# rmcolq/charon

Measured on AMD Instinct MI355X. Metric: classified reads/sec + achieved HBM GB/s vs roofline, 5 kb reads, 39 GB index, higher is better.
Workload: dtype u64

## Files before the change

charon_amd/api.py:

```python
import ctypes as C
import os

import numpy as np

HERE = os.path.dirname(os.path.abspath(__file__))
LIB_PATH = os.environ.get("CHARON_HIP_LIB") or os.path.join(HERE, "libcharon_hip.so")
if not os.path.exists(LIB_PATH):
    raise ImportError("charon_amd: %s not built -- run `python -c 'import __graft_entry__ as g; g.build()'`" % LIB_PATH)
_L = C.CDLL(LIB_PATH)

MINIMISER_SEED = 0x8F3F73B5CF1C9ADE
STREAM_PROFILE = 1
STREAM_TINY_LOG = 2
GZIP_TALLIES, GZIP_SIZES, GZIP_BOTH = 0, 1, 2
GZIP_SIZES_ALL = 3
GZIP_ANY_LEN = 0xFFFFFFFF


class IndexDesc(C.Structure):
    _fields_ = [("struct_size", C.c_uint32), ("device", C.c_int32), ("kmer_size", C.c_uint8), ("window_size", C.c_uint8),
                ("hash_funs", C.c_uint8), ("num_categories", C.c_uint8), ("host_index", C.c_uint8), ("reserved0", C.c_uint8 * 3),
                ("minimiser_seed", C.c_uint64), ("bins", C.c_uint64), ("technical_bins", C.c_uint64), ("bin_size", C.c_uint64),
                ("hash_shift", C.c_uint64), ("bin_words", C.c_uint64), ("bin_to_category", C.c_uint8 * 256),
                ("row_begin", C.c_uint64), ("row_end", C.c_uint64)]


class Model(C.Structure):
    _fields_ = [("struct_size", C.c_uint32), ("num_categories", C.c_uint32), ("pos_data", C.POINTER(C.POINTER(C.c_float))),
                ("pos_n", C.POINTER(C.c_uint32)), ("neg_data", C.POINTER(C.POINTER(C.c_float))), ("neg_n", C.POINTER(C.c_uint32)),
                ("h_pos", C.c_float), ("h_neg", C.c_float), ("err_rate", C.c_float), ("min_quality", C.c_float),
                ("min_length", C.c_uint32), ("min_compression", C.c_float), ("confidence_threshold", C.c_int8),
                ("min_hits", C.c_uint8), ("paired", C.c_uint8), ("host_index", C.c_uint8),
                ("confidence_probability_threshold", C.c_float), ("host_unique_prop_lo_threshold", C.c_float),
                ("min_proportion_difference", C.c_float), ("min_prob_difference", C.c_float),
                ("dist", C.c_uint32), ("pos_params", C.POINTER(C.c_float)), ("neg_params", C.POINTER(C.c_float))]


class StreamCfg(C.Structure):
    _fields_ = [("struct_size", C.c_uint32), ("flags", C.c_uint32), ("max_reads", C.c_uint64), ("max_bases", C.c_uint64)]


class Batch(C.Structure):
    _fields_ = [("struct_size", C.c_uint32), ("on_device", C.c_uint32), ("n_reads", C.c_uint64), ("n_bases", C.c_uint64),
                ("bases2", C.c_void_p), ("nmask", C.c_void_p), ("seg1_offset", C.c_void_p), ("seg1_length", C.c_void_p),
                ("seg2_offset", C.c_void_p), ("seg2_length", C.c_void_p), ("mean_quality", C.c_void_p),
                ("compression", C.c_void_p), ("gzip_tallies", C.c_uint32), ("gzip_output", C.c_uint32)]
# ... 288 lines not shown

    def synth_fill(self, seed, density):
        _chk(_L.chn_synth_fill_index(self.h, seed, density))

    def synth_plant(self, dev_genomes, n_genomes, genome_len, genome_bin):
        _chk(_L.chn_synth_plant(self.h, dev_genomes, n_genomes, genome_len, bytes(bytearray(int(b) for b in genome_bin))))

    def destroy(self):
        if self.h:
            _L.chn_index_destroy(self.h)
            self.h = None


DIST = {"kde": 0, "gamma": 1, "beta": 2}
DIST_DEFAULTS = {"gamma": ((25.0, 0.0, 0.02), (10.0, 0.0, 0.005)), "beta": ((6.0, 4.0, 0.0), (6.0, 40.0, 0.0))}


def default_model(num_categories, host_index, paired=False, dist="kde", pos_params=None, neg_params=None, **overrides):
    m = Model()
    _chk(_L.chn_model_default(C.byref(m), num_categories, host_index, 1 if paired else 0))
    if dist != "kde":
        pp = np.ascontiguousarray(pos_params if pos_params is not None else [DIST_DEFAULTS[dist][0]] * num_categories, np.float32)
        nn = np.ascontiguousarray(neg_params if neg_params is not None else [DIST_DEFAULTS[dist][1]] * num_categories, np.float32)
        m._keep = (pp, nn)
        m.dist = DIST[dist]
        m.pos_params = pp.ctypes.data_as(C.POINTER(C.c_float))
        m.neg_params = nn.ctypes.data_as(C.POINTER(C.c_float))
    for k, v in overrides.items():
        setattr(m, k, v)
    return m


class Stream:
    def __init__(self, index, max_reads, max_bases, profile=False, tiny_log=False, split_bucket=0):
        self.index = index
        cfg = StreamCfg(C.sizeof(StreamCfg), (STREAM_PROFILE if profile else 0) | (STREAM_TINY_LOG if tiny_log else 0) | ((split_bucket & 0xff) << 8),
                        max_reads, max_bases)
        self.h = C.c_void_p()
        _chk(_L.chn_stream_create(index.h, C.byref(cfg), C.byref(self.h)))
        self.C = index.desc.num_categories
        self._fifo = []

    def set_model(self, model):
        _chk(_L.chn_model_set(self.h, C.byref(model)))

    def submit_host(self, packed, mean_quality=None, compression=None, gzip_tallies=0, gzip_output=0):
        b, keep, n = self._host_batch(packed, mean_quality, compression)
        b.gzip_tallies, b.gzip_output = gzip_tallies, gzip_output
        _chk(_L.chn_batch_submit(self.h, C.byref(b)))
        self._fifo.append((n, keep, gzip_tallies, gzip_output))

    def _host_batch(self, packed, mean_quality, compression):
        n = len(packed["seg1_length"])
        b = Batch()
        b.struct_size, b.on_device, b.n_reads, b.n_bases = C.sizeof(Batch), 0, n, packed["n_bases"]
        keep = []

        def ptr(a, dt):
            if a is None:
                return None
            a = np.ascontiguousarray(a, dtype=dt)
            keep.append(a)
            return a.ctypes.data

        b.bases2 = ptr(packed["bases2"], np.uint32)
        b.nmask = ptr(packed.get("nmask"), np.uint32)
        b.seg1_offset = ptr(packed["seg1_offset"], np.uint64)
        b.seg1_length = ptr(packed["seg1_length"], np.uint32)
        b.seg2_offset = ptr(packed.get("seg2_offset"), np.uint64)
# ... 638 lines not shown
```

charon_amd/csrc/parts/abi_index_model.inc:

```

struct chn_index {
    chn_index_desc d;
    uint64_t *words = nullptr;
    uint64_t rows_local = 0;
    bool single_bin_categories = false;
    hipStream_t ef_stream = nullptr;
    hipEvent_t ef_copied = nullptr;
    void *ef_buf[2][4] = {{nullptr, nullptr, nullptr, nullptr}, {nullptr, nullptr, nullptr, nullptr}};
    size_t ef_cap[2][4] = {{0, 0, 0, 0}, {0, 0, 0, 0}};
    unsigned long long *ef_bad = nullptr;
    unsigned ef_turn = 0;
    void ef_release() {
        if (ef_stream) (void)hipStreamSynchronize(ef_stream);
        for (int k = 0; k < 2; ++k)
            for (int i = 0; i < 4; ++i) { if (ef_buf[k][i]) (void)hipFree(ef_buf[k][i]); ef_buf[k][i] = nullptr; ef_cap[k][i] = 0; }
        if (ef_bad) (void)hipFree(ef_bad);
        ef_bad = nullptr;
        if (ef_copied) (void)hipEventDestroy(ef_copied);
        ef_copied = nullptr;
        if (ef_stream) (void)hipStreamDestroy(ef_stream);
        ef_stream = nullptr;
    }
};

// ... 136 lines not shown
    chn_stream_cfg cfg;
    hipStream_t stream = nullptr;
    hipStream_t stream1 = nullptr;
    hipStream_t stream2 = nullptr;
    hipStream_t stream0 = nullptr;
    hipStream_t stream3 = nullptr;
    hipStream_t stream4 = nullptr;
    hipStream_t stream5 = nullptr;
    uint32_t long_bucket = 104;
    DevBuf d_hist, d_model;
    DevBuf d_memo;
    LogBuf big;
    DevBuf d_list, d_cbase;
    uint64_t shard_entries = 0;
    bool shard_open = false;
    LogBuf shx;
    DevBuf d_shx_cnt;
    ShxArgs shx_args;
    int shx_stage = 0;
    uint32_t cap_num = 65536, esc_shift = 0;
    uint64_t overflow_reruns = 0;
    bool gzt_big_lds = false;
    DevBuf d_gzscratch;
    DevBuf d_gzlscratch[2];
    bool gzl_big_lds = false;
    uint32_t n_cus = 256;
    static const int N_SLOTS = 3;
    Slot slot[N_SLOTS];
    PinBuf h_block;
    int head = 0;
    int inflight = 0;
    uint64_t batch_seq = 0;
    bool last_had_long = false;
    HostModel model;
    K3Args k3;
    struct CountsBufs { DevBuf num_hashes, counts, unique, len1, mq, comp, prob, call, conf, flags; } cc;
    double prof_ms[4] = {0, 0, 0, 0};
    uint64_t prof_n[4] = {0, 0, 0, 0};
    hipEvent_t prof_anchor[2] = {nullptr, nullptr};
    int prof_cur = 0;
    bool prof_anchor_pending = false, prof_have_end = false;
    double prof_prev_end = 0;
    std::chrono::steady_clock::time_point prof_anchor_at;
    uint64_t last_bytes = 0, last_min = 0, last_fetches = 0;
    double text_ms[2] = {0, 0};
    uint64_t text_n = 0;
    TextSplitScratch tsp;
    TextFetchScratch txg;
    TextPairScratch tpi;
};

static uint64_t pow5(unsigned e) { uint64_t p = 1; while (e--) p *= 5; return p; }

extern "C" int chn_index_create(const chn_index_desc *desc, chn_index **out) {
    if (!desc || !out || desc->struct_size != sizeof(chn_index_desc)) return fail(CHN_E_INVALID, "chn_index_create: bad descriptor");
    const chn_index_desc &d = *desc;
    if (d.kmer_size < 1 || d.kmer_size > 27) return fail(CHN_E_INVALID, "kmer_size must be in 1..27 (5^k has to fit 64 bits)");
    if (d.window_size < d.kmer_size) return fail(CHN_E_INVALID, "window_size must be >= kmer_size");
    if (d.hash_funs < 1 || d.hash_funs > 5) return fail(CHN_E_INVALID, "hash_funs must be in 1..5");
    if (d.bins < 1 || d.bins > 255 || d.technical_bins != ((d.bins + 63) / 64) * 64 || d.bin_words != d.technical_bins / 64)
        return fail(CHN_E_INVALID, "IBF header inconsistent: technical_bins must be 64*ceil(bins/64), bin_words = technical_bins/64");
    if (d.bin_size == 0 || d.hash_shift != (uint64_t)__builtin_clzll(d.bin_size)) return fail(CHN_E_INVALID, "hash_shift must be countl_zero(bin_size)");
    if (d.num_categories < 1) return fail(CHN_E_INVALID, "num_categories must be >= 1");
    for (uint64_t b = 0; b < d.bins; ++b)
        if (d.bin_to_category[b] >= d.num_categories) return fail(CHN_E_INVALID, "bin_to_category entry out of range");
    chn_index *idx = new (std::nothrow) chn_index();
// ... 283 lines not shown
```

charon_amd/csrc/parts/abi_shard_wait.inc:

```

static int ensure_shard_buffers(chn_stream *s) {
    const uint64_t nw = (s->cfg.max_reads + WAVE - 1) / WAVE;
    int rc;
    if ((rc = s->big.ensure(s->cfg.max_bases, nw, (uint32_t)s->idx->d.bin_words, 65536, 0))) return rc;
    if ((rc = s->d_list.ensure(s->big.log_cap * 8)) || (rc = s->d_cbase.ensure((nw + 1) * 8))) return rc;
    return CHN_OK;
}
static ShardArgs shard_args(chn_stream *s, const chn_index *shard, uint64_t *partial, const Slot &sl) {
    ShardArgs a;
    std::memset(&a, 0, sizeof a);
    const chn_index_desc &d = shard->d;
    a.list = s->d_list.as<uint64_t>(); a.wave_meta = s->big.meta.as<WaveMeta>(); a.cbase = s->d_cbase.as<uint64_t>();
    a.wave_count = s->big.wcount.as<uint32_t>(); a.words = shard->words; a.S = d.bin_size; a.row_begin = d.row_begin; a.row_end = d.row_end;
    a.shift = (uint32_t)d.hash_shift; a.h = d.hash_funs; a.W = (uint32_t)d.bin_words; a.partial = partial; a.rows = s->big.rows.as<uint64_t>();
    a.rowlog = s->big.log.as<uint32_t>(); a.B = (uint32_t)d.bins;
    a.n_waves = (uint32_t)((sl.n_reads + WAVE - 1) / WAVE); a.esc_capacity = s->big.esc_cap;
    a.status = reinterpret_cast<uint32_t *>(const_cast<Slot &>(sl).d_ctl.as<unsigned long long>() + CTL_STATUS);
    return a;
}

extern "C" int chn_shard_minimise(chn_stream *s, const chn_batch *b, uint64_t *n_entries) {
    if (!s || !b || !n_entries) return fail(CHN_E_INVALID, "chn_shard_minimise: null argument");
    if (s->shard_open) return fail(CHN_E_STATE, "chn_shard_minimise: previous sharded batch not finished");
    HIPCHK(hipSetDevice(s->idx->d.device));
// ... 103 lines not shown
    HIPCHK(hipStreamWaitEvent(s->stream2, sl.k1_done, 0));
    int rc = launch_tail(s, sl, s->big, s->stream2);
    if (rc) return rc;
    s->head = (s->head + 1) % chn_stream::N_SLOTS;
    s->inflight += 1;
    return CHN_OK;
}

extern "C" int chn_stream_sync(chn_stream *s) {
    if (!s) return fail(CHN_E_INVALID, "null stream");
    HIPCHK(hipSetDevice(s->idx->d.device));
    HIPCHK(hipStreamSynchronize(s->stream0));
    HIPCHK(hipStreamSynchronize(s->stream));
    HIPCHK(hipStreamSynchronize(s->stream1));
    HIPCHK(hipStreamSynchronize(s->stream4));
    HIPCHK(hipStreamSynchronize(s->stream2));
    return CHN_OK;
}

static int rerun_worst_case(chn_stream *s, Slot &sl) {
    const chn_index_desc &d = s->idx->d;
    unsigned long long *ctl = sl.d_ctl.as<unsigned long long>();
    const uint64_t n = sl.n_reads, nw = (n + WAVE - 1) / WAVE + sl.split_bound;
    HIPCHK(hipMemsetAsync(ctl, 0, CTL_NLONG * 8, s->stream));
    HIPCHK(hipMemsetAsync(ctl + CTL_FETCHES, 0, (CTL_WORDS - CTL_FETCHES) * 8, s->stream));
    hipLaunchKernelGGL(k_sum_len, dim3((uint32_t)std::min<uint64_t>(1024, (n + 255) / 256)), dim3(256), 0, s->stream, sl.len1, sl.len2, (uint32_t)n, ctl + CTL_WORDS - 1);
    HIPCHK(hipGetLastError());
    unsigned long long total = 0;
    HIPCHK(hipMemcpyAsync(&total, ctl + CTL_WORDS - 1, 8, hipMemcpyDeviceToHost, s->stream));
    HIPCHK(hipStreamSynchronize(s->stream));
    int rc = s->big.ensure(total, (n + WAVE - 1) / WAVE + std::min<uint64_t>(sl.split_bound, total / len_bucket_floor(std::min(s->long_bucket, 247u)) + 1), (uint32_t)d.bin_words, 65536, 0, nw);
    if (rc) return rc;
    K1Args a = sl.k1;
    fill_k1_log(a, sl, s->big, true);
    const size_t lds = k1_lds_bytes(a.wn, d.num_categories, MODE_ROWS, a.h, (uint32_t)d.bin_words, (uint32_t)d.bins);
    hipError_t e = launch_k1_mode(MODE_ROWS, (uint32_t)d.bin_words, a, lds, s->stream);
    if (e == hipSuccess && sl.split_bound) e = launch_k1_split_mode(MODE_ROWS, (uint32_t)d.bin_words, a, lds, s->stream, split_grid(sl.split_bound));
    if (e != hipSuccess) return fail(CHN_E_HIP, std::string("k_minimise_probe re-run: ") + hipGetErrorString(e));
    if ((rc = launch_tail(s, sl, s->big, s->stream))) return rc;
    HIPCHK(hipStreamSynchronize(s->stream));
    s->overflow_reruns += 1;
    return CHN_OK;
}

extern "C" int chn_batch_wait(chn_stream *s, chn_result *r) {
    if (!s || !r || r->struct_size != sizeof(chn_result)) return fail(CHN_E_INVALID, "chn_batch_wait: bad argument");
    if (s->inflight == 0) return fail(CHN_E_STATE, "no batch in flight");
    HIPCHK(hipSetDevice(s->idx->d.device));
    Slot &sl = s->slot[(s->head + chn_stream::N_SLOTS - s->inflight) % chn_stream::N_SLOTS];
    static const bool diag_wait = diag_env("CHN_DIAG_WAIT") != nullptr;
    auto dnow = []() { return std::chrono::duration<double>(std::chrono::steady_clock::now().time_since_epoch()).count(); };
    const double dw0 = diag_wait ? dnow() : 0;
    HIPCHK(hipEventSynchronize(sl.done));
    const double dw1 = diag_wait ? dnow() : 0;
    if (sl.want_gzt) HIPCHK(hipEventSynchronize(sl.gz_done));
    const double dw2 = diag_wait ? dnow() : 0;
    struct DiagPrint { bool on; double a, b, c; std::function<double()> now; ~DiagPrint() { if (on) std::fprintf(stderr, "chn_batch_wait: at %.4f  done-event %.2f ms  gz-event %.2f ms  rest %.2f ms\n", a, (b - a) * 1e3, (c - b) * 1e3, (now() - c) * 1e3); } } diag_print{diag_wait, dw0, dw1, dw2, dnow};
    s->inflight -= 1;
    static const int evpair[4][2] = {{0, 1}, {2, 3}, {4, 5}, {6, 7}};
    for (int i = 0; i < 4; ++i)
        if (sl.ev_used[i]) {
            float ms = 0;
            HIPCHK(hipEventElapsedTime(&ms, sl.ev[evpair[i][0]], sl.ev[evpair[i][1]]));
            if (i == 0) {
                float t0 = 0, t1 = 0;
                HIPCHK(hipEventElapsedTime(&t0, s->prof_anchor[s->prof_cur], sl.ev[0]));
// ... 111 lines not shown
    k3.mean_quality = mean_quality ? b.mq.as<float>() : nullptr; k3.compression = compression ? b.comp.as<float>() : nullptr;
    k3.prob = b.prob.as<double>(); k3.call = b.call.as<uint8_t>(); k3.conf = b.conf.as<uint8_t>(); k3.flags = b.flags.as<uint8_t>();
    k3.n_reads = (uint32_t)n;
    hipLaunchKernelGGL(k_model_call, dim3((uint32_t)((n + 255) / 256)), dim3(256), 0, s->stream, k3);
    HIPCHK(hipGetLastError());
    HIPCHK(hipStreamSynchronize(s->stream));
    HIPCHK(hipMemcpy(probabilities, b.prob.p, n * C * 8, hipMemcpyDeviceToHost));
    HIPCHK(hipMemcpy(call, b.call.p, n, hipMemcpyDeviceToHost));
    HIPCHK(hipMemcpy(confidence, b.conf.p, n, hipMemcpyDeviceToHost));
    HIPCHK(hipMemcpy(flags, b.flags.p, n, hipMemcpyDeviceToHost));
    return CHN_OK;
}

extern "C" int chn_classify_counts(chn_stream *s, uint64_t n, const uint32_t *num_hashes, const uint32_t *counts,
                                   const uint32_t *unique_counts, const uint32_t *lengths, const float *mean_quality,
                                   const float *compression, double *probabilities, uint8_t *call, uint8_t *confidence) {
    std::vector<uint8_t> flags(std::max<uint64_t>(n, 1));
    int rc = chn_classify_counts_raw(s, n, num_hashes, counts, unique_counts, lengths, mean_quality, compression, probabilities, call,
                                     confidence, flags.data());
    if (rc) return rc;
    const uint64_t C = s->idx->d.num_categories;
    std::vector<double> p(C);
    const bool all = s->model.dist != CHN_DIST_KDE;
    for (uint64_t i = 0; i < n; ++i)
        if (all || flags[i] || num_hashes[i] == 0) {
            host_model_call(s->model, num_hashes[i], counts + i * C, unique_counts + i * C, mean_quality ? mean_quality[i] : 0.0f,
                            compression ? compression[i] : 0.0f, lengths[i], p.data(), &call[i], &confidence[i]);
            for (uint64_t c = 0; c < C; ++c) probabilities[i * C + c] = p[c];
        }
    return CHN_OK;
}

extern "C" int chn_stream_profile(chn_stream *s, int which, double *total_ms, uint64_t *launches, int reset) {
    if (!s || which < 0 || which > 11 || which == 10) return fail(CHN_E_INVALID, "chn_stream_profile: bad argument");
    if (which == 11) {
        if (total_ms) *total_ms = s->tpi.ms;
        if (launches) *launches = s->tpi.calls;
        if (reset) { s->tpi.ms = 0; s->tpi.calls = 0; }
        return CHN_OK;
    }
    if (which == 9) {
        if (total_ms) *total_ms = s->txg.ms;
        if (launches) *launches = s->txg.calls;
        if (reset) { s->txg.ms = 0; s->txg.calls = 0; }
        return CHN_OK;
    }
    if (which == 8) {
        if (total_ms) *total_ms = s->tsp.ms;
        if (launches) *launches = s->tsp.calls;
        if (reset) { s->tsp.ms = 0; s->tsp.calls = 0; }
        return CHN_OK;
    }
    if (which >= 6) {
        if (total_ms) *total_ms = s->text_ms[which - 6];
        if (launches) *launches = s->text_n;
        if (reset) { s->text_ms[which - 6] = 0; if (which == 7) s->text_n = 0; }
        return CHN_OK;
    }
    if (which == 5) {
        if (total_ms) *total_ms = 0;
        if (launches) *launches = s->last_fetches;
        return CHN_OK;
    }
    if (which == 4) {
        if (total_ms) *total_ms = 0;
        if (launches) *launches = s->overflow_reruns;
        if (reset) s->overflow_reruns = 0;
// ... 21 lines not shown
```

charon_amd/csrc/parts/abi_stream_batch.inc:

```

struct ResLayout {
    size_t ctl, prob, nh, counts, unique, call, conf, flags, total;
    ResLayout(uint64_t n, uint64_t C) {
        ctl = 0; prob = CTL_WORDS * 8; nh = prob + n * C * 8; counts = nh + n * 4; unique = counts + n * C * 4; call = unique + n * C * 4;
        conf = call + n; flags = conf + n; total = flags + n;
    }
};

static const int PROF_ANCHOR_SECONDS = 8;
static hipError_t prof_anchor_now(chn_stream *s) {
    for (Slot &sl : s->slot) sl.new_anchor = false;
    s->prof_cur = 0; s->prof_anchor_pending = false; s->prof_have_end = false; s->prof_prev_end = 0;
    hipError_t e = hipEventRecord(s->prof_anchor[0], s->stream);
    if (e == hipSuccess) e = hipEventSynchronize(s->prof_anchor[0]);
    s->prof_anchor_at = std::chrono::steady_clock::now();
    return e;
}

extern "C" int chn_stream_create(chn_index *idx, const chn_stream_cfg *cfg, chn_stream **out) {
    if (!idx || !cfg || !out || cfg->struct_size != sizeof(chn_stream_cfg)) return fail(CHN_E_INVALID, "chn_stream_create: bad argument");
    if (cfg->max_reads == 0 || cfg->max_reads > 0xFFFFFF00ULL) return fail(CHN_E_INVALID, "max_reads out of range");
    HIPCHK(hipSetDevice(idx->d.device));
    idx->ef_release();
    chn_stream *s = new (std::nothrow) chn_stream();
    if (!s) return fail(CHN_E_NOMEM, "host allocation failed");
    s->idx = idx; s->cfg = *cfg;
    int prio_least = 0, prio_greatest = 0;
    hipError_t e = hipDeviceGetStreamPriorityRange(&prio_least, &prio_greatest);
    if (e == hipSuccess) e = hipStreamCreateWithFlags(&s->stream, hipStreamNonBlocking);
    if (e == hipSuccess) e = hipStreamCreateWithFlags(&s->stream1, hipStreamNonBlocking);
    if (e == hipSuccess) e = hipStreamCreateWithPriority(&s->stream2, hipStreamNonBlocking, prio_greatest);
    if (e == hipSuccess) e = hipStreamCreateWithPriority(&s->stream0, hipStreamNonBlocking, prio_greatest);
    if (e == hipSuccess) e = hipStreamCreateWithPriority(&s->stream3, hipStreamNonBlocking, prio_least);
    if (e == hipSuccess) e = hipStreamCreateWithFlags(&s->stream4, hipStreamNonBlocking);
    {
        const uint32_t ob = (cfg->flags >> 8) & 0xffu;
        s->long_bucket = ob == 0 ? LONG_BUCKET_DEFAULT : ob == 255 ? 256u : std::max(64u, ob);
    }
    if (e != hipSuccess) { chn_stream_destroy(s); return fail(CHN_E_HIP, std::string("hipStreamCreate: ") + hipGetErrorString(e)); }
    const uint64_t n = cfg->max_reads, C = idx->d.num_categories;
    int rc = CHN_OK;
    const bool sharded = idx->d.row_begin != 0 || idx->d.row_end != idx->d.bin_size;
    const bool fused = !sharded && idx->single_bin_categories && C <= 8 && idx->d.bin_words == 1;
    const uint32_t wn = (uint32_t)idx->d.window_size - idx->d.kmer_size + 1;
    s->cap_num = (uint32_t)std::min<uint64_t>(65536, (4ULL * 65536 + wn) / (wn + 1));
    s->esc_shift = idx->d.bins <= 128 ? 3u : 1u;
    if (cfg->flags & CHN_STREAM_TINY_LOG) { s->cap_num = 64; s->esc_shift = 6; }
    const uint64_t nw = (n + WAVE - 1) / WAVE + (s->long_bucket < 256 ? std::min<uint64_t>(n, cfg->max_bases / len_bucket_floor(s->long_bucket)) : 0);
    for (Slot &sl : s->slot) {
        for (int i = 0; i < 8 && e == hipSuccess; ++i) e = hipEventCreate(&sl.ev[i]);
        if (e == hipSuccess) e = hipEventCreateWithFlags(&sl.k1_done, hipEventDisableTiming);
        if (e == hipSuccess) e = hipEventCreateWithFlags(&sl.split_done, hipEventDisableTiming);
        if (e == hipSuccess) e = hipEventCreateWithFlags(&sl.done, hipEventDisableTiming);
        if (e == hipSuccess) e = hipEventCreateWithFlags(&sl.uploaded, hipEventDisableTiming);
        if (e == hipSuccess) e = hipEventCreateWithFlags(&sl.bases_up, hipEventDisableTiming);
        if (e == hipSuccess) e = hipEventCreateWithFlags(&sl.gz_done, hipEventDisableTiming);
        if (e == hipSuccess) e = hipEventCreateWithFlags(&sl.gzt_done, hipEventDisableTiming);
        if (e != hipSuccess) { chn_stream_destroy(s); return fail(CHN_E_HIP, std::string("hipEventCreate: ") + hipGetErrorString(e)); }
        if ((rc = sl.d_num_hashes.ensure(n * 4)) || (rc = sl.d_counts.ensure(n * C * 4)) || (rc = sl.d_unique.ensure(n * C * 4)) ||
            (rc = sl.d_prob.ensure(n * C * 8)) || (rc = sl.d_call.ensure(n)) || (rc = sl.d_conf.ensure(n)) || (rc = sl.d_flags.ensure(n)) ||
            (rc = sl.d_ctl.ensure(CTL_WORDS * 8)) || (rc = sl.d_order.ensure(n * 4))) {
            chn_stream_destroy(s);
            return rc;
        }
        if (!fused && !sharded && (rc = sl.lb.ensure(cfg->max_bases, nw, (uint32_t)idx->d.bin_words, s->cap_num, s->esc_shift, (n + WAVE - 1) / WAVE + n))) { chn_stream_destroy(s); return rc; }
    }
    if ((rc = s->d_hist.ensure(LEN_BLOCKS * 256 * 4))) { chn_stream_destroy(s); return rc; }
    if (cfg->flags & CHN_STREAM_PROFILE) {
        for (hipEvent_t &a : s->prof_anchor) if (e == hipSuccess) e = hipEventCreate(&a);
        if (e == hipSuccess) e = prof_anchor_now(s);
        if (e != hipSuccess) { chn_stream_destroy(s); return fail(CHN_E_HIP, std::string("profiling anchor: ") + hipGetErrorString(e)); }
    }
    {
        int cus = 0;
        if (hipDeviceGetAttribute(&cus, hipDeviceAttributeMultiprocessorCount, idx->d.device) == hipSuccess && cus > 0) s->n_cus = (uint32_t)cus;
    }
    {
        const size_t res = (ResLayout(n, C).total + 255) & ~(size_t)255, gzs = (n * 4 + 255) & ~(size_t)255;
        if ((res + gzs) * chn_stream::N_SLOTS <= ((size_t)64 << 20) && s->h_block.ensure((res + gzs) * chn_stream::N_SLOTS) == CHN_OK) {
            char *base = s->h_block.as<char>();
            for (int i = 0; i < chn_stream::N_SLOTS; ++i) {
                s->slot[i].h_res.lend(base + (size_t)i * (res + gzs), res);
                s->slot[i].h_gzsize.lend(base + (size_t)i * (res + gzs) + res, gzs);
            }
        }
    }
    *out = s;
    return CHN_OK;
}

extern "C" int chn_stream_destroy(chn_stream *s) {
    if (!s) return CHN_OK;
    (void)hipSetDevice(s->idx->d.device);
    if (s->stream) { (void)hipStreamSynchronize(s->stream); }
    if (s->stream1) { (void)hipStreamSynchronize(s->stream1); (void)hipStreamDestroy(s->stream1); }
    if (s->stream2) { (void)hipStreamSynchronize(s->stream2); (void)hipStreamDestroy(s->stream2); }
    if (s->stream0) { (void)hipStreamSynchronize(s->stream0); (void)hipStreamDestroy(s->stream0); }
    if (s->stream3) { (void)hipStreamSynchronize(s->stream3); (void)hipStreamDestroy(s->stream3); }
    if (s->stream4) { (void)hipStreamSynchronize(s->stream4); (void)hipStreamDestroy(s->stream4); }
    if (s->stream5) { (void)hipStreamSynchronize(s->stream5); (void)hipStreamDestroy(s->stream5); }
    if (s->stream) (void)hipStreamDestroy(s->stream);
    for (hipEvent_t a : s->prof_anchor) if (a) (void)hipEventDestroy(a);
    for (Slot &sl : s->slot) {
        for (int i = 0; i < 8; ++i) if (sl.ev[i]) (void)hipEventDestroy(sl.ev[i]);
        if (sl.k1_done) (void)hipEventDestroy(sl.k1_done);
        if (sl.split_done) (void)hipEventDestroy(sl.split_done);
        if (sl.done) (void)hipEventDestroy(sl.done);
        if (sl.uploaded) (void)hipEventDestroy(sl.uploaded);
        if (sl.bases_up) (void)hipEventDestroy(sl.bases_up);
        if (sl.gz_done) (void)hipEventDestroy(sl.gz_done);
        if (sl.gzt_done) (void)hipEventDestroy(sl.gzt_done);
        sl.h_res.release(); sl.h_gzt.release(); sl.h_gzsize.release(); sl.d_gzsize.release();
        sl.h_text.release(); sl.d_text.release(); sl.d_tdesc.release(); sl.d_tctl.release();
        for (int i = 0; i < 4; ++i) if (sl.tev[i]) (void)hipEventDestroy(sl.tev[i]);
        s->h_block.release();
        DevBuf *bufs[] = {&sl.d_num_hashes, &sl.d_counts, &sl.d_unique, &sl.d_prob, &sl.d_call, &sl.d_conf, &sl.d_flags, &sl.d_ctl, &sl.d_order, &sl.d_gzt, &sl.d_gzidx, &sl.d_gzctr, &sl.d_gzlong,
                          &sl.d_len1, &sl.d_len2, &sl.d_mq, &sl.d_comp, &sl.d_bases, &sl.d_nmask, &sl.d_off1, &sl.d_off2};
        for (DevBuf *b : bufs) b->release();
        sl.lb.release();
    }
    DevBuf *bufs[] = {&s->d_hist, &s->d_model, &s->d_list, &s->d_cbase, &s->d_memo, &s->d_shx_cnt, &s->d_gzscratch, &s->d_gzlscratch[0], &s->d_gzlscratch[1],
                      &s->cc.num_hashes, &s->cc.counts, &s->cc.unique, &s->cc.len1, &s->cc.mq, &s->cc.comp, &s->cc.prob, &s->cc.call,
                      &s->cc.conf, &s->cc.flags};
    for (DevBuf *b : bufs) b->release();
    s->big.release();
    s->shx.release();
    s->tsp.release();
    s->txg.release();
    s->tpi.release();
    delete s;
    return CHN_OK;
}

extern "C" int chn_model_set(chn_stream *s, const chn_model *m) {
// ... 416 lines not shown
    a.bases = bases; a.nmask = nmask; a.off1 = off1; a.off2 = off2; a.len1 = sl.len1; a.len2 = sl.len2; a.n_bases = b->n_bases;
    a.order = sl.d_order.as<uint32_t>();
    a.status = reinterpret_cast<uint32_t *>(ctl + CTL_STATUS);
    if (const char *ab = diag_env("CHN_ABLATE")) a.ablate = (uint32_t)std::atoi(ab);
    a.nt_probes = s->idx->rows_local * d.bin_words * 8 > (4ULL << 30) ? 1u : 0u;
    if (const char *nt = diag_env("CHN_NT_PROBES")) a.nt_probes = (uint32_t)std::atoi(nt);
    a.num_hashes = sl.d_num_hashes.as<uint32_t>(); a.counts = sl.d_counts.as<uint32_t>(); a.unique = sl.d_unique.as<uint32_t>();
    const uint32_t n_waves = (uint32_t)((n + WAVE - 1) / WAVE);
    a.n_long_ptr = sl.split_bound ? ctl + CTL_NLONG : nullptr; a.wave_slot0 = n_waves;
    a.fetches = ctl + CTL_FETCHES;
    if (list_kind == LIST_SPARSE) {
        fill_k1_log(a, sl, s->shx, true);
        a.rows = s->d_list.as<uint64_t>();
    } else if (list_mode) {
        fill_k1_log(a, sl, s->big, false);
        a.rows = s->d_list.as<uint64_t>();
        hipLaunchKernelGGL(k_wave_caps, dim3((uint32_t)((n + 255) / 256)), dim3(256), 0, ps, sl.d_order.as<uint32_t>(), sl.len1, sl.len2,
                           (uint32_t)n, s->big.cap_num, s->big.esc_shift, s->big.meta.as<WaveMeta>());
        hipLaunchKernelGGL(k_scan_meta, dim3(1), dim3(1024), 0, ps, s->big.meta.as<WaveMeta>(), n_waves);
        HIPCHK(hipGetLastError());
    } else if (!fused) {
        fill_k1_log(a, sl, sl.lb, true);
    }
    const int mode = list_mode ? MODE_LIST : fused ? MODE_FUSED : MODE_ROWS;
    size_t lds = k1_lds_bytes(a.wn, C, mode, a.h, W, a.B);
    if (const char *pad = diag_env("CHN_LDS_PAD")) lds += (size_t)std::atoi(pad);
    if (lds > 160 * 1024) return fail(CHN_E_INVALID, "window too large for LDS");
    if (sl.split_bound) {
        HIPCHK(hipStreamWaitEvent(s->stream4, sl.uploaded, 0));
        hipError_t e4 = launch_k1_split_mode(mode, W, a, lds, s->stream4, split_grid(sl.split_bound));
        if (e4 != hipSuccess) return fail(CHN_E_HIP, std::string("k_minimise_probe (split) launch: ") + hipGetErrorString(e4));
        HIPCHK(hipEventRecord(sl.split_done, s->stream4));
    }
    if (prof) { HIPCHK(hipEventRecord(sl.ev[0], ps)); }
    hipError_t e = launch_k1_mode(mode, W, a, lds, ps);
    if (e != hipSuccess) return fail(CHN_E_HIP, std::string("k_minimise_probe launch: ") + hipGetErrorString(e));
    if (prof) {
        if (sl.split_bound) HIPCHK(hipStreamWaitEvent(ps, sl.split_done, 0));
        HIPCHK(hipEventRecord(sl.ev[1], ps)); sl.ev_used[0] = true;
        if (!s->prof_anchor_pending && std::chrono::steady_clock::now() - s->prof_anchor_at > std::chrono::seconds(PROF_ANCHOR_SECONDS)) {
            HIPCHK(hipEventRecord(s->prof_anchor[s->prof_cur ^ 1], ps));
            s->prof_anchor_at = std::chrono::steady_clock::now();
            sl.new_anchor = s->prof_anchor_pending = true;
        }
    }

    if (list_mode) return CHN_OK;
    dt[3] = dnow();
    HIPCHK(hipEventRecord(sl.k1_done, ps));
    HIPCHK(hipStreamWaitEvent(s->stream2, sl.k1_done, 0));
    if (sl.split_bound) HIPCHK(hipStreamWaitEvent(s->stream2, sl.split_done, 0));
    int rc = launch_tail(s, sl, sl.lb, s->stream2);
    if (rc) return rc;
    if (diag_sub) std::fprintf(stderr, "submit: validate + uploads %.2f ms, deflate tallies %.2f, ordering + probe launch %.2f, tail %.2f\n",
                               (dt[1] - dt[0]) * 1e3, (dt[2] - dt[1]) * 1e3, (dt[3] - dt[2]) * 1e3, (dnow() - dt[3]) * 1e3);
    s->head = (s->head + 1) % chn_stream::N_SLOTS;
    s->inflight += 1;
    s->batch_seq += 1;
    return CHN_OK;
}


static int launch_tail(chn_stream *s, Slot &sl, LogBuf &lb, hipStream_t st) {
    const chn_index_desc &d = s->idx->d;
    const uint64_t n = sl.n_reads;
    const uint32_t W = (uint32_t)d.bin_words, C = d.num_categories;
    const uint32_t n_waves = (uint32_t)((n + WAVE - 1) / WAVE);
    const bool prof = (s->cfg.flags & CHN_STREAM_PROFILE) != 0 && st == s->stream2;
    unsigned long long *ctl = sl.d_ctl.as<unsigned long long>();
    if (!sl.fused) {
        K2Args k2;
        std::memset(&k2, 0, sizeof(k2));
        k2.rows = lb.rows.as<uint64_t>(); k2.rowlog = lb.log.as<uint32_t>();
        k2.wave_meta = lb.meta.as<WaveMeta>(); k2.wave_count = lb.wcount.as<uint32_t>(); k2.order = sl.d_order.as<uint32_t>();
        k2.counts = sl.d_counts.as<uint32_t>(); k2.unique = sl.d_unique.as<uint32_t>();
        k2.n_reads = (uint32_t)n; k2.B = (uint32_t)d.bins; k2.C = C; k2.W = W;
        std::memcpy(k2.b2c, d.bin_to_category, 256);
        k2.n_long_ptr = sl.split_bound && !sl.list_mode ? ctl + CTL_NLONG : nullptr; k2.wave_slot0 = n_waves;
        const dim3 grid(n_waves), block(K2_THREADS);
        const bool t16 = !sl.list_mode && sl.len2 == nullptr && s->long_bucket <= LONG_BUCKET_DEFAULT;
        uint32_t G = WAVE;
        while (G > 8 && k2_lds_bytes((uint32_t)d.bins, C, W, G, t16) > K2_LDS_BUDGET) G >>= 1;
        k2.group = G;
        const size_t lds2 = k2_lds_bytes((uint32_t)d.bins, C, W, G, t16);
// ... 73 lines not shown
```

charon_amd/csrc/parts/k1_minimise_probe.inc:

```

enum { MODE_FUSED = 0, MODE_ROWS = 1, MODE_EMPLACE = 2, MODE_LIST = 3 };
#ifndef CHN_LOG_BATCH
#define CHN_LOG_BATCH 4
#endif
#ifndef CHN_BASE_PIECES
#define CHN_BASE_PIECES 4
#endif

#ifndef K1_COND_MAX_BINS
#define K1_COND_MAX_BINS 4u
#endif
#ifndef FUSED_ROUNDS
#define FUSED_ROUNDS 2u
#endif

struct WaveMeta { uint64_t base, esc_base; uint32_t cap, esc_cap, pad0, pad1; };

struct K1Args {
    const uint64_t *words;
    uint64_t *words_rw;
    uint64_t S, row_begin, row_end, seed, powk1;
    uint32_t shift, h, k, wn, n_reads, nseg, B, C;
    uint64_t b2c_packed;
    const uint32_t *bases, *nmask;
    const uint64_t *off1, *off2;
    const uint32_t *len1, *len2;
    const uint32_t *order;
    uint32_t *num_hashes, *counts, *unique;
    uint64_t *rows;
    uint32_t *rowlog;
    WaveMeta *wave_meta;
    uint32_t *wave_count;
    unsigned long long *cursor;
    uint64_t log_capacity, esc_capacity;
    uint32_t cap_num, esc_shift;
    uint32_t *status;
    uint64_t n_bases;
    uint32_t nt_probes;
    const uint8_t *read_bin;
    uint32_t ablate;
    const unsigned long long *n_long_ptr;
    uint32_t wave_slot0;
    unsigned long long *fetches;
};

__device__ bool first_window_tied(const K1Args &a, uint64_t o, uint32_t wn) {
    const uint64_t INV5 = 0xCCCCCCCCCCCCCCCDULL;
    const uint32_t k = a.k, w = wn + k - 1;
    uint64_t fwd = 0, rc = 0, best = ~0ULL;
    bool tie = false;
    auto digits = [&](uint64_t x, uint32_t &d, uint32_t &cd) {
        const uint32_t code = (a.bases[x >> 4] >> ((x & 15u) * 2u)) & 3u;
        const uint32_t nf = a.nmask ? (a.nmask[x >> 5] >> (x & 31u)) & 1u : 0u;
        d = nf ? 3u : code + (code == 3u);
        cd = nf ? 3u : (3u - code) + (code == 0u);
    };
    for (uint32_t i = 0; i < w; ++i) {
        uint32_t d_in, cd_in, d_out = 0, cd_out = 0;
        digits(o + i, d_in, cd_in);
        if (i >= k) digits(o + i - k, d_out, cd_out);
        fwd = (fwd - (uint64_t)d_out * a.powk1) * 5u + d_in;
        rc = (rc - cd_out) * INV5 + (uint64_t)cd_in * a.powk1;
        if (i + 1 >= k) {
            const uint64_t vf = fwd ^ a.seed, vr = rc ^ a.seed, v = vf < vr ? vf : vr;
            if (v < best) { best = v; tie = false; } else if (v == best) tie = true;
        }
    }
    return tie;
}

#define ROWLOG_ESC_MASK 0x03fffffcu
#define ROWLOG_ESC_MAX 0x00fffffeu
__host__ __device__ __forceinline__ uint64_t wave_log_cap(uint64_t sum_len, uint32_t cap_num) { return (((sum_len * cap_num) >> 16) + 64 + 63) & ~63ULL; }
__host__ __device__ __forceinline__ uint64_t wave_esc_cap(uint64_t cap, uint32_t esc_shift) { return (cap >> esc_shift) + 64; }
template <int W>
__device__ __forceinline__ uint32_t encode_row(const uint64_t *acc, uint32_t B, uint32_t owner, bool &escaped) {
    uint64_t m[W];
// ... 19 lines not shown
    }
    return e;
}

__device__ __forceinline__ void lds_dma_b128(const void *src, uint32_t lds_dst, bool nt) {
    unsigned keep;
    const uint32_t dst = (uint32_t)__builtin_amdgcn_readfirstlane((int)lds_dst);
    if (nt)
        asm volatile("s_mov_b32 %0, m0\n\ts_mov_b32 m0, %2\n\ts_nop 0\n\tglobal_load_lds_dwordx4 %1, off nt\n\ts_mov_b32 m0, %0"
                     : "=&s"(keep) : "v"(src), "s"(dst) : "memory");
    else
        asm volatile("s_mov_b32 %0, m0\n\ts_mov_b32 m0, %2\n\ts_nop 0\n\tglobal_load_lds_dwordx4 %1, off\n\ts_mov_b32 m0, %0"
                     : "=&s"(keep) : "v"(src), "s"(dst) : "memory");
}
__device__ __forceinline__ void wait_vmcnt(uint32_t n) {
    switch (n) {
        case 0: asm volatile("s_waitcnt vmcnt(0)" ::: "memory"); break;
        case 1: asm volatile("s_waitcnt vmcnt(1)" ::: "memory"); break;
        case 2: asm volatile("s_waitcnt vmcnt(2)" ::: "memory"); break;
        case 3: asm volatile("s_waitcnt vmcnt(3)" ::: "memory"); break;
        case 4: asm volatile("s_waitcnt vmcnt(4)" ::: "memory"); break;
        case 5: asm volatile("s_waitcnt vmcnt(5)" ::: "memory"); break;
        case 6: asm volatile("s_waitcnt vmcnt(6)" ::: "memory"); break;
        case 7: asm volatile("s_waitcnt vmcnt(6)" ::: "memory"); break;
        case 8: asm volatile("s_waitcnt vmcnt(8)" ::: "memory"); break;
        case 9: asm volatile("s_waitcnt vmcnt(8)" ::: "memory"); break;
        default: asm volatile("s_waitcnt vmcnt(10)" ::: "memory"); break;
    }
}

template <int W, int MODE, int WN_T, bool SPLIT = false, bool COND_T = false>
__global__ __launch_bounds__(WAVE) void k_minimise_probe(const K1Args a) {
    extern __shared__ __align__(16) unsigned char smem[];
    const uint32_t n_long = a.n_long_ptr ? (uint32_t)__builtin_nontemporal_load(a.n_long_ptr) : 0u;
    uint32_t item = blockIdx.x;
    if (SPLIT && item >= n_long) return;
    do {
    const uint32_t wslot = SPLIT ? a.wave_slot0 + item : item;
    const uint32_t wn = WN_T ? (uint32_t)WN_T : a.wn;
    constexpr uint32_t NBLK = (W == 1 || W == 2) ? 1u : 2u;
    constexpr bool COND = MODE == MODE_FUSED && COND_T;
    constexpr uint32_t QC = COND ? QCAP + WAVE : QCAP;
    auto qwrap = [&](uint32_t x) -> uint32_t {
        if (!COND) return x & (QC - 1);
        x = x >= QC ? x - QC : x;
        return x >= QC ? x - QC : x;
    };
    const uint32_t pb_round = COND ? 1024u : (MODE == MODE_FUSED || MODE == MODE_ROWS) ? a.h * NBLK * 1024u : 0u;
    unsigned char *pbuf = smem;
    const uint32_t pbuf_lds = (uint32_t)(size_t)(__attribute__((address_space(3))) unsigned char *)smem;
    uint64_t *ring = reinterpret_cast<uint64_t *>(smem + (COND ? FUSED_ROUNDS : 2u) * pb_round);
    uint64_t *qv = ring + (size_t)wn * WAVE;
    uint64_t *qa = qv + QC;
    uint32_t *qm = reinterpret_cast<uint32_t *>(qa + (COND ? QC : 0u));
    uint64_t *rbase = reinterpret_cast<uint64_t *>(qm + QC);
    uint32_t *cnt = reinterpret_cast<uint32_t *>(rbase + (MODE == MODE_EMPLACE ? WAVE : 0));
    uint32_t *unq = cnt + (MODE == MODE_FUSED ? a.C * WAVE : 0);
    uint8_t *spos = reinterpret_cast<uint8_t *>(unq + (MODE == MODE_FUSED ? a.C * WAVE : 0));
    uint32_t *sbuf = reinterpret_cast<uint32_t *>(smem + (((size_t)(spos + (size_t)wn * WAVE - smem) + 15) & ~(size_t)15));

    const uint32_t lane = lane_id();
    const uint32_t g = SPLIT ? item : item * WAVE + lane;
    const bool valid = SPLIT ? true : (g < a.n_reads && g >= n_long);
    const uint32_t r = valid ? (a.order ? a.order[g] : g) : 0;
    const uint32_t own = SPLIT ? 0u : lane;
    bool cold = false;
// ... 608 lines not shown
```

charon_amd/csrc/parts/len_order.inc:

```

__device__ __forceinline__ uint32_t len_bucket(uint32_t len) {
    if (len < 8) return len;
    const uint32_t e = 31u - (uint32_t)__clz((int)len);
    return (e - 2) * 8 + ((len >> (e - 3)) & 7u);
}
#define LEN_BLOCKS 256
enum { CTL_BYTES = 0, CTL_MINIMISERS = 1, CTL_LOG_CURSOR = 2, CTL_ESC_CURSOR = 3, CTL_STATUS = 4, CTL_NLONG = 5, CTL_FETCHES = 6, CTL_WORDS = 8 };
#define LONG_BUCKET_DEFAULT 104u
__host__ __device__ __forceinline__ uint32_t len_bucket_floor(uint32_t bucket) {
    const uint32_t e = bucket / 8 + 2, sub = bucket & 7u;
    return (1u << e) + (sub << (e - 3));
}
__global__ __launch_bounds__(256) void k_len_hist(const uint32_t *len1, const uint32_t *len2, uint32_t n, uint32_t *blockhist ,
                                                  unsigned long long *ctl) {
    __shared__ uint32_t sh[256];
    sh[threadIdx.x] = 0;
    if (blockIdx.x == 0 && threadIdx.x < CTL_WORDS) ctl[threadIdx.x] = 0;
    __syncthreads();
    const uint32_t chunk = (n + LEN_BLOCKS - 1) / LEN_BLOCKS, lo = blockIdx.x * chunk, hi = min(n, lo + chunk);
    for (uint32_t i = lo + threadIdx.x; i < hi; i += 256) atomicAdd(&sh[len_bucket(len1[i] + (len2 ? len2[i] : 0u))], 1u);
    __syncthreads();
    blockhist[blockIdx.x * 256 + threadIdx.x] = sh[threadIdx.x];
}
__global__ __launch_bounds__(256) void k_len_scatter(const uint32_t *len1, const uint32_t *len2, uint32_t n, const uint32_t *blockhist, uint32_t *order,
                                                     unsigned long long *ctl, uint32_t long_bucket, uint32_t split_cap) {
    __shared__ uint32_t cursor[256], tot[256];
    __shared__ uint16_t tile[256];
    {
        const uint32_t b = threadIdx.x;
        uint32_t t = 0, pre = 0;
        for (uint32_t k = 0; k < LEN_BLOCKS; ++k) { const uint32_t c = blockhist[k * 256 + b]; t += c; if (k < blockIdx.x) pre += c; }
        tot[b] = t;
        __syncthreads();
        uint32_t start = 0;
        for (uint32_t x = b + 1; x < 256; ++x) start += tot[x];
        cursor[b] = start + pre;
        if (blockIdx.x == 0 && b == long_bucket && !len2 && start + tot[b] <= split_cap) ctl[CTL_NLONG] = (unsigned long long)start + tot[b];
    }
    const uint32_t chunk = (n + LEN_BLOCKS - 1) / LEN_BLOCKS, lo = blockIdx.x * chunk, hi = min(n, lo + chunk);
    for (uint32_t base = lo; base < hi; base += 256) {
// ... 38 lines not shown
```

include/charon_hip.h:

```cpp
#ifndef CHARON_HIP_H
#define CHARON_HIP_H

#include <stddef.h>
#include <stdint.h>

#ifdef __cplusplus
extern "C" {
#endif

#define CHN_OK 0
#define CHN_E_INVALID (-1)
#define CHN_E_HIP (-2)
#define CHN_E_NOMEM (-3)
#define CHN_E_STATE (-4)
#define CHN_E_CAPACITY (-5)

#define CHN_MAX_CATEGORIES 255
#define CHN_NO_CALL 255u

typedef struct chn_index chn_index;
typedef struct chn_stream chn_stream;

typedef struct chn_index_desc {
    uint32_t struct_size;
// ... 36 lines not shown
    const uint32_t *neg_n;
    float h_pos;
    float h_neg;
    float err_rate;
    float min_quality;
    uint32_t min_length;
    float min_compression;
    int8_t confidence_threshold;
    uint8_t min_hits;
    uint8_t paired;
    uint8_t host_index;
    float confidence_probability_threshold;
    float host_unique_prop_lo_threshold;
    float min_proportion_difference;
    float min_prob_difference;
    uint32_t dist;
    const float *pos_params;
    const float *neg_params;
} chn_model;
#define CHN_DIST_KDE 0u
#define CHN_DIST_GAMMA 1u
#define CHN_DIST_BETA 2u

int chn_model_default(chn_model *m, uint32_t num_categories, uint8_t host_index, int paired);

typedef struct chn_stream_cfg {
    uint32_t struct_size;
    uint32_t flags;
    uint64_t max_reads;
    uint64_t max_bases;
} chn_stream_cfg;
#define CHN_STREAM_PROFILE 1u
#define CHN_STREAM_TINY_LOG 2u
#define CHN_STREAM_SPLIT_BUCKET(b) (((uint32_t)(b) & 0xffu) << 8)

int chn_stream_create(chn_index *idx, const chn_stream_cfg *cfg, chn_stream **out);
int chn_stream_destroy(chn_stream *s);
int chn_model_set(chn_stream *s, const chn_model *m);

typedef struct chn_batch {
    uint32_t struct_size;
    uint32_t on_device;
    uint64_t n_reads;
    uint64_t n_bases;
    const uint32_t *bases2;
    const uint32_t *nmask;
    const uint64_t *seg1_offset;
    const uint32_t *seg1_length;
    const uint64_t *seg2_offset;
    const uint32_t *seg2_length;
    const float *mean_quality;
    const float *compression;
    uint32_t gzip_tallies;
    uint32_t gzip_output;
} chn_batch;
#define CHN_GZIP_TALLIES 0u
#define CHN_GZIP_SIZES 1u
#define CHN_GZIP_BOTH 2u
#define CHN_GZIP_SIZES_ALL 3u
#define CHN_GZIP_ANY_LEN 0xFFFFFFFFu
#define CHN_GZIP_MAX_LEN 61440u
#define CHN_GZIP_TALLY_WORDS 320u

typedef struct chn_result {
    uint32_t struct_size;
    uint32_t on_device;
// ... 214 lines not shown
```

Before: 33.31 million.

## Gate probe kernel launches on alternate streams with a device signal

Adds a device-side signal that makes each batch's minimise/probe kernel on the alternating stream wait with hipStreamWaitValue64 until the previous batch's probe kernel has dispatched all its blocks (or finished). The first block to see the full grid started bumps the signal, and a release kernel bumps it again after completion. The aim is to stop two probe kernels from interleaving and thrashing HBM or cache on the 39 GB index while still allowing some overlap. This adds an atomic per block, a stream wait and an extra tiny kernel per batch, and concurrency drops when the gate stalls.

```diff
diff --git a/charon_amd/api.py b/charon_amd/api.py
--- a/charon_amd/api.py
+++ b/charon_amd/api.py
@@ -12,6 +12,7 @@
 MINIMISER_SEED = 0x8F3F73B5CF1C9ADE
 STREAM_PROFILE = 1
 STREAM_TINY_LOG = 2
+STREAM_NO_PROBE_GATE = 4
 GZIP_TALLIES, GZIP_SIZES, GZIP_BOTH = 0, 1, 2
 GZIP_SIZES_ALL = 3
 GZIP_ANY_LEN = 0xFFFFFFFF
@@ -366,9 +367,10 @@
 
 
 class Stream:
-    def __init__(self, index, max_reads, max_bases, profile=False, tiny_log=False, split_bucket=0):
+    def __init__(self, index, max_reads, max_bases, profile=False, tiny_log=False, split_bucket=0, probe_gate=True):
         self.index = index
-        cfg = StreamCfg(C.sizeof(StreamCfg), (STREAM_PROFILE if profile else 0) | (STREAM_TINY_LOG if tiny_log else 0) | ((split_bucket & 0xff) << 8),
+        cfg = StreamCfg(C.sizeof(StreamCfg), (STREAM_PROFILE if profile else 0) | (STREAM_TINY_LOG if tiny_log else 0) | (0 if probe_gate else STREAM_NO_PROBE_GATE) |
+                        ((split_bucket & 0xff) << 8),
                         max_reads, max_bases)
         self.h = C.c_void_p()
         _chk(_L.chn_stream_create(index.h, C.byref(cfg), C.byref(self.h)))
diff --git a/charon_amd/csrc/parts/abi_index_model.inc b/charon_amd/csrc/parts/abi_index_model.inc
--- a/charon_amd/csrc/parts/abi_index_model.inc
+++ b/charon_amd/csrc/parts/abi_index_model.inc
@@ -192,6 +192,9 @@
     int inflight = 0;
     uint64_t batch_seq = 0;
     bool last_had_long = false;
+    unsigned long long *gate_signal = nullptr;
+    uint64_t gate_seq = 0;
+    uint64_t gated_batches = 0;
     HostModel model;
     K3Args k3;
     struct CountsBufs { DevBuf num_hashes, counts, unique, len1, mq, comp, prob, call, conf, flags; } cc;
diff --git a/charon_amd/csrc/parts/abi_shard_wait.inc b/charon_amd/csrc/parts/abi_shard_wait.inc
--- a/charon_amd/csrc/parts/abi_shard_wait.inc
+++ b/charon_amd/csrc/parts/abi_shard_wait.inc
@@ -159,6 +159,7 @@
     int rc = s->big.ensure(total, (n + WAVE - 1) / WAVE + std::min<uint64_t>(sl.split_bound, total / len_bucket_floor(std::min(s->long_bucket, 247u)) + 1), (uint32_t)d.bin_words, 65536, 0, nw);
     if (rc) return rc;
     K1Args a = sl.k1;
+    a.gate_started = a.gate_signal = nullptr;
     fill_k1_log(a, sl, s->big, true);
     const size_t lds = k1_lds_bytes(a.wn, d.num_categories, MODE_ROWS, a.h, (uint32_t)d.bin_words, (uint32_t)d.bins);
     hipError_t e = launch_k1_mode(MODE_ROWS, (uint32_t)d.bin_words, a, lds, s->stream);
@@ -336,7 +337,13 @@
 }
 
 extern "C" int chn_stream_profile(chn_stream *s, int which, double *total_ms, uint64_t *launches, int reset) {
-    if (!s || which < 0 || which > 11 || which == 10) return fail(CHN_E_INVALID, "chn_stream_profile: bad argument");
+    if (!s || which < 0 || which > 13 || which == 10 || which == 12) return fail(CHN_E_INVALID, "chn_stream_profile: bad argument");
+    if (which == 13) {
+        if (total_ms) *total_ms = s->gate_signal ? 1.0 : 0.0;
+        if (launches) *launches = s->gated_batches;
+        if (reset) s->gated_batches = 0;
+        return CHN_OK;
+    }
     if (which == 11) {
         if (total_ms) *total_ms = s->tpi.ms;
         if (launches) *launches = s->tpi.calls;
diff --git a/charon_amd/csrc/parts/abi_stream_batch.inc b/charon_amd/csrc/parts/abi_stream_batch.inc
--- a/charon_amd/csrc/parts/abi_stream_batch.inc
+++ b/charon_amd/csrc/parts/abi_stream_batch.inc
@@ -38,6 +38,16 @@
         s->long_bucket = ob == 0 ? LONG_BUCKET_DEFAULT : ob == 255 ? 256u : std::max(64u, ob);
     }
     if (e != hipSuccess) { chn_stream_destroy(s); return fail(CHN_E_HIP, std::string("hipStreamCreate: ") + hipGetErrorString(e)); }
+    {
+        int can_wait = 0;
+        const char *off = diag_env("CHN_PROBE_GATE");
+        if (!(cfg->flags & CHN_STREAM_NO_PROBE_GATE) && !(off && std::atoi(off) == 0) &&
+            hipDeviceGetAttribute(&can_wait, hipDeviceAttributeCanUseStreamWaitValue, idx->d.device) == hipSuccess && can_wait) {
+            e = hipExtMallocWithFlags((void **)&s->gate_signal, 8, hipMallocSignalMemory);
+            if (e == hipSuccess) e = hipMemset(s->gate_signal, 0, 8);
+            if (e != hipSuccess) { chn_stream_destroy(s); return fail(CHN_E_HIP, std::string("probe gate signal: ") + hipGetErrorString(e)); }
+        }
+    }
     const uint64_t n = cfg->max_reads, C = idx->d.num_categories;
     int rc = CHN_OK;
     const bool sharded = idx->d.row_begin != 0 || idx->d.row_end != idx->d.bin_size;
@@ -100,6 +110,7 @@
     if (s->stream4) { (void)hipStreamSynchronize(s->stream4); (void)hipStreamDestroy(s->stream4); }
     if (s->stream5) { (void)hipStreamSynchronize(s->stream5); (void)hipStreamDestroy(s->stream5); }
     if (s->stream) (void)hipStreamDestroy(s->stream);
+    if (s->gate_signal) (void)hipFree(s->gate_signal);
     for (hipEvent_t a : s->prof_anchor) if (a) (void)hipEventDestroy(a);
     for (Slot &sl : s->slot) {
         for (int i = 0; i < 8; ++i) if (sl.ev[i]) (void)hipEventDestroy(sl.ev[i]);
@@ -582,9 +593,18 @@
         if (e4 != hipSuccess) return fail(CHN_E_HIP, std::string("k_minimise_probe (split) launch: ") + hipGetErrorString(e4));
         HIPCHK(hipEventRecord(sl.split_done, s->stream4));
     }
+    const bool gated = !list_mode && alternate && s->gate_signal != nullptr;
+    if (gated) {
+        if (s->gate_seq) {
+            HIPCHK(hipStreamWaitValue64(ps, s->gate_signal, s->gate_seq, hipStreamWaitValueGte, ~0ull));
+            s->gated_batches += 1;
+        }
+        a.gate_started = ctl + CTL_GATE; a.gate_signal = s->gate_signal; a.gate_value = s->gate_seq + 1;
+    }
     if (prof) { HIPCHK(hipEventRecord(sl.ev[0], ps)); }
     hipError_t e = launch_k1_mode(mode, W, a, lds, ps);
     if (e != hipSuccess) return fail(CHN_E_HIP, std::string("k_minimise_probe launch: ") + hipGetErrorString(e));
+    if (gated) s->gate_seq += 1;
     if (prof) {
         if (sl.split_bound) HIPCHK(hipStreamWaitEvent(ps, sl.split_done, 0));
         HIPCHK(hipEventRecord(sl.ev[1], ps)); sl.ev_used[0] = true;
@@ -600,6 +620,10 @@
     HIPCHK(hipEventRecord(sl.k1_done, ps));
     HIPCHK(hipStreamWaitEvent(s->stream2, sl.k1_done, 0));
     if (sl.split_bound) HIPCHK(hipStreamWaitEvent(s->stream2, sl.split_done, 0));
+    if (gated) {
+        hipLaunchKernelGGL(k_gate_release, dim3(1), dim3(1), 0, ps, s->gate_signal, (unsigned long long)s->gate_seq);
+        HIPCHK(hipGetLastError());
+    }
     int rc = launch_tail(s, sl, sl.lb, s->stream2);
     if (rc) return rc;
     if (diag_sub) std::fprintf(stderr, "submit: validate + uploads %.2f ms, deflate tallies %.2f, ordering + probe launch %.2f, tail %.2f\n",
diff --git a/charon_amd/csrc/parts/k1_minimise_probe.inc b/charon_amd/csrc/parts/k1_minimise_probe.inc
--- a/charon_amd/csrc/parts/k1_minimise_probe.inc
+++ b/charon_amd/csrc/parts/k1_minimise_probe.inc
@@ -42,7 +42,14 @@
     const unsigned long long *n_long_ptr;
     uint32_t wave_slot0;
     unsigned long long *fetches;
+    unsigned long long *gate_started, *gate_signal;
+    unsigned long long gate_value;
 };
+__global__ void k_gate_release(unsigned long long *signal, unsigned long long value) {
+    if (threadIdx.x == 0 && blockIdx.x == 0) [[clang::atomic(remote_memory, fine_grained_memory)]] {
+        (void)__hip_atomic_fetch_max(signal, value, __ATOMIC_RELAXED, __HIP_MEMORY_SCOPE_SYSTEM);
+    }
+}
 
 __device__ bool first_window_tied(const K1Args &a, uint64_t o, uint32_t wn) {
     const uint64_t INV5 = 0xCCCCCCCCCCCCCCCDULL;
@@ -128,6 +135,11 @@
 template <int W, int MODE, int WN_T, bool SPLIT = false, bool COND_T = false>
 __global__ __launch_bounds__(WAVE) void k_minimise_probe(const K1Args a) {
     extern __shared__ __align__(16) unsigned char smem[];
+    if (!SPLIT && a.gate_started && threadIdx.x == 0) {
+        if (atomicAdd(a.gate_started, 1ULL) == (unsigned long long)gridDim.x - 1) [[clang::atomic(remote_memory, fine_grained_memory)]] {
+            (void)__hip_atomic_fetch_max(a.gate_signal, a.gate_value, __ATOMIC_RELAXED, __HIP_MEMORY_SCOPE_SYSTEM);
+        }
+    }
     const uint32_t n_long = a.n_long_ptr ? (uint32_t)__builtin_nontemporal_load(a.n_long_ptr) : 0u;
     uint32_t item = blockIdx.x;
     if (SPLIT && item >= n_long) return;
diff --git a/charon_amd/csrc/parts/len_order.inc b/charon_amd/csrc/parts/len_order.inc
--- a/charon_amd/csrc/parts/len_order.inc
+++ b/charon_amd/csrc/parts/len_order.inc
@@ -5,7 +5,7 @@
     return (e - 2) * 8 + ((len >> (e - 3)) & 7u);
 }
 #define LEN_BLOCKS 256
-enum { CTL_BYTES = 0, CTL_MINIMISERS = 1, CTL_LOG_CURSOR = 2, CTL_ESC_CURSOR = 3, CTL_STATUS = 4, CTL_NLONG = 5, CTL_FETCHES = 6, CTL_WORDS = 8 };
+enum { CTL_BYTES = 0, CTL_MINIMISERS = 1, CTL_LOG_CURSOR = 2, CTL_ESC_CURSOR = 3, CTL_STATUS = 4, CTL_NLONG = 5, CTL_FETCHES = 6, CTL_GATE = 7, CTL_WORDS = 8 };
 #define LONG_BUCKET_DEFAULT 104u
 __host__ __device__ __forceinline__ uint32_t len_bucket_floor(uint32_t bucket) {
     const uint32_t e = bucket / 8 + 2, sub = bucket & 7u;
diff --git a/include/charon_hip.h b/include/charon_hip.h
--- a/include/charon_hip.h
+++ b/include/charon_hip.h
@@ -92,6 +92,7 @@
 } chn_stream_cfg;
 #define CHN_STREAM_PROFILE 1u
 #define CHN_STREAM_TINY_LOG 2u
+#define CHN_STREAM_NO_PROBE_GATE 4u
 #define CHN_STREAM_SPLIT_BUCKET(b) (((uint32_t)(b) & 0xffu) << 8)
 
 int chn_stream_create(chn_index *idx, const chn_stream_cfg *cfg, chn_stream **out);
```

Result: faster. 34.10 million, median of 6 (+2.4%).
